# Terascale-All-sensing-Research-Studio/MOV-SLAM

Hardware: AMD Instinct MI355X
Metric: local-BA iterations/sec (50 KF x 20k MapPoint window) (higher is better)
Workload: dtype f64; 1 GPU; LocalBundleAdjustment 50 KF + 10 fixed x 20000 MapPoints, E=110510 mono edges, Huber on, 10 LM iterations (cfg3, seed 1003); one window per GPU; parallelism=1 window

## Files before the change

### mov-slam_amd/csrc/coarse_level.h

```cpp
#pragma once
#include <hip/hip_runtime.h>

#include <type_traits>

#include "device_math.h"
#include "device_types.h"
#include "handoff.h"

namespace movba {

#ifndef MOVBA_COARSE_EXTRAPOLATE
#define MOVBA_COARSE_EXTRAPOLATE 1
#endif

template <int kT, int kNC, int kPA>
__device__ __forceinline__ void coarse_build(const DevWindow &w, const PcgParams &pp, int trial, double lambda, double *sm, bool extrapolate)
{
    double *Ac = sm;
    double *gj = Ac + kNC * kNC;
    int &s_bad = *reinterpret_cast<int *>(gj + 9 * kNC + 2);
    const int tid = threadIdx.x;
    const int nf = w.nfree;
#ifdef MOVBA_CLOCK_STAMP
    unsigned long long cst_last = __builtin_amdgcn_s_memtime();
#define COARSE_STAMP(k) do { const unsigned long long _t = __builtin_amdgcn_s_memtime(); if (tid == 0) w.ctrl->dbg_seg2[k] += _t - cst_last; cst_last = _t; } while (0)
#else
#define COARSE_STAMP(k) do { } while (0)
#endif
    const double *part = w.part, *part_ = part;
    double *blocks = w.blocks_c;
    if (tid == 0) s_bad = 0;
    for (int idx = tid; idx < kNC * kNC; idx += kT) Ac[idx] = 0.0;

    const int ndiag = nf * 36;
    for (int idx = tid; idx < w.n_multi * 36; idx += kT) {
        const int m = idx / 36, k = idx - m * 36, pr = w.multi_pairs[m];
        double sacc = 0.0;
        for (int itx = w.pair_item_start[pr]; itx < w.pair_item_start[pr + 1]; ++itx) sacc += part[(size_t)itx * kPartStride + k];
        blocks[pr * 36 + k] = -sacc;
    }
    for (int base = tid; base < ndiag; base += 4 * kT) {
        int k[4], hu[4], i0[4], i1[4];
        double s[4] = { 0, 0, 0, 0 }, hp[4] = { 0, 0, 0, 0 };
        int nmax = 0;
#pragma unroll
        for (int m = 0; m < 4; ++m) {
            const int idx = min(base + m * kT, ndiag - 1);
            const int pr = idx / 36;
            k[m] = idx - pr * 36;
            const int a = k[m] / 6, b = k[m] - a * 6;
            hu[m] = 42 + (a <= b ? ut6(a, b) : ut6(b, a));
            i0[m] = w.pair_item_start[pr]; i1[m] = w.pair_item_start[pr + 1];
            nmax = max(nmax, i1[m] - i0[m]);
        }
        for (int o = 0; o < nmax; o += 6) {
            double sv[4][6], hv[4][6];
#pragma unroll
            for (int m = 0; m < 4; ++m)
#pragma unroll
                for (int u = 0; u < 6; ++u) {
                    const double *src = part + (size_t)min(i0[m] + o + u, i1[m] - 1) * kPartStride;
                    sv[m][u] = src[k[m]]; hv[m][u] = src[hu[m]];
                }
#pragma unroll
            for (int m = 0; m < 4; ++m)
#pragma unroll
                for (int u = 0; u < 6; ++u) { const bool in = i0[m] + o + u < i1[m]; s[m] += in ? sv[m][u] : 0.0; hp[m] += in ? hv[m][u] : 0.0; }
        }
#pragma unroll
        for (int m = 0; m < 4; ++m) {
            const int idx = base + m * kT;
            if (idx < ndiag) blocks[idx] = (hp[m] + ((k[m] % 7 == 0) ? lambda : 0.0)) - s[m];
        }
    }
    __syncthreads();
    COARSE_STAMP(2);
    double *aggc = gj;
    if (tid < kNC / kPA) {
        const int g0 = pp.wave_row0[tid], g1 = pp.wave_row0[tid + 1];
        aggc[tid] = g0 + 0.5 * (g1 - g0 - 1); aggc[kNC / kPA + tid] = 1.0 / fmax(1.0, 0.5 * (g1 - g0));
    }
    int *tent = reinterpret_cast<int *>(gj + 9 * kNC + 8), *tij = tent + w.cblk_ptr[w.n_cblk];
    for (int q = tid; q < w.cblk_ptr[w.n_cblk]; q += kT) { tent[q] = w.cblk_ent[q]; tij[q] = w.cblk_ij[q]; }
    __syncthreads();
    const int nw = w.n_cblk * 6;
    const bool split = 2 * nw <= kT;
    auto walk = [&](int cb, int a, int part, double (&s00)[6], double (&s01)[6], double (&s10)[6], double (&s11)[6]) {
        const int g = w.cblk_g[cb], h = w.cblk_h[cb];
        const double cg = aggc[g], ch = aggc[h], ig = aggc[kNC / kPA + g], ih = aggc[kNC / kPA + h];
        int t0 = w.cblk_ptr[cb], t1 = w.cblk_ptr[cb + 1];
        if (split) {
            const int n = t1 - t0, front = min(n, (((n + 1) >> 1) + 7) & ~7);
            if (part == 0) t1 = t0 + front; else t0 += front;
        }
#pragma unroll
        for (int m = 0; m < 6; ++m) s00[m] = s01[m] = s10[m] = s11[m] = 0.0;
        for (int t = t0; t < t1; t += 8) {
            int pk[8], ij[8];
            double v[8][6];
#pragma unroll
            for (int u = 0; u < 8; ++u) { const int tt = min(t + u, t1 - 1); pk[u] = tent[tt]; ij[u] = tij[tt]; }
#pragma unroll
            for (int u = 0; u < 8; ++u) {
                const int e = pk[u];
                const double *src = (e & 1) ? part_ + (size_t)(e >> 2) * kPartStride : blocks + (size_t)(e >> 2) * 36;
                const int o0 = (e & 2) ? a : a * 6, st = (e & 2) ? 6 : 1;
#pragma unroll
                for (int m = 0; m < 6; ++m) v[u][m] = src[o0 + st * m];
            }
#pragma unroll
            for (int u = 0; u < 8; ++u) {
                const bool in = t + u < t1;
                const double sgn = in ? ((pk[u] & 1) ? -1.0 : 1.0) : 0.0;
                const double pi = ((ij[u] >> 16) - cg) * ig, pj = ((ij[u] & 0xffff) - ch) * ih;
#pragma unroll
                for (int m = 0; m < 6; ++m) {
                    const double x = sgn * v[u][m];
                    s00[m] += x; s01[m] += pj * x; s10[m] += pi * x; s11[m] += pi * pj * x;
                }
            }
        }
        return Ac + (g * kPA + a) * kNC + h * kPA;
    };
    if (split) {
        const bool active = tid < 2 * nw;
        const int half = tid >= nw, wi = tid - half * nw;
        double s00[6], s01[6], s10[6], s11[6];
        double *dst = nullptr;
        if (active) dst = walk(wi / 6, wi - (wi / 6) * 6, half, s00, s01, s10, s11);
        if (active && !half) {
#pragma unroll
            for (int m = 0; m < 6; ++m) { dst[m] = s00[m]; dst[6 + m] = s01[m]; dst[6 * kNC + m] = s10[m]; dst[6 * kNC + 6 + m] = s11[m]; }
        }
        __syncthreads();
        if (active && half) {
#pragma unroll
            for (int m = 0; m < 6; ++m) { dst[m] += s00[m]; dst[6 + m] += s01[m]; dst[6 * kNC + m] += s10[m]; dst[6 * kNC + 6 + m] += s11[m]; }
        }
    } else {
        for (int wi = tid; wi < nw; wi += kT) {
            double s00[6], s01[6], s10[6], s11[6];
            double *dst = walk(wi / 6, wi - (wi / 6) * 6, 0, s00, s01, s10, s11);
#pragma unroll
            for (int m = 0; m < 6; ++m) { dst[m] = s00[m]; dst[6 + m] = s01[m]; dst[6 * kNC + m] = s10[m]; dst[6 * kNC + 6 + m] = s11[m]; }
        }
    }
    __syncthreads();
    if (tid < kNC) {
        const int g = tid / kPA, d = (tid - g * kPA) / 6, nrows = pp.wave_row0[g + 1] - pp.wave_row0[g];
        if (nrows == 0 || (d == 1 && nrows < 2)) {
            for (int j = 0; j < kNC; ++j) { Ac[tid * kNC + j] = 0.0; Ac[j * kNC + tid] = 0.0; }
        }
    }
    __syncthreads();
    if (tid < kNC) {
        const int g = tid / kPA, d = (tid - g * kPA) / 6, nrows = pp.wave_row0[g + 1] - pp.wave_row0[g];
        if (nrows == 0 || (d == 1 && nrows < 2)) Ac[tid * kNC + tid] = 1.0;
    }
    __syncthreads();
    if (extrapolate) {
        double *prev = w.ac_prev;
        const double lam_prev = prev[kNC * kNC], trial_prev = prev[kNC * kNC + 1];
        double gamma = 0.0;
        if (trial >= 1 && trial_prev == (double)(trial - 1) && lambda != lam_prev && MOVBA_COARSE_EXTRAPOLATE) {
            gamma = (lambda * (1.0 / 3.0) - lambda) / (lambda - lam_prev);
            gamma = fmin(fmax(gamma, -1.0), 1.0 / 3.0);
            if (!isfinite(gamma)) gamma = 0.0;
        }
        constexpr int kPer = kNC * kNC / kT;
        static_assert(kPer * kT == kNC * kNC, "one pass");
        double pv[kPer];
#pragma unroll
        for (int u = 0; u < kPer; ++u) pv[u] = prev[tid + u * kT];
        __syncthreads();
#pragma unroll
        for (int u = 0; u < kPer; ++u) {
            const double a = Ac[tid + u * kT];
            prev[tid + u * kT] = a;
            if (gamma != 0.0) Ac[tid + u * kT] = a + gamma * (a - pv[u]);
        }
        if (tid == 0) { prev[kNC * kNC] = lambda; prev[kNC * kNC + 1] = (double)trial; }
        __syncthreads();
    }

    COARSE_STAMP(3);
    static_assert(kNC == 96 && kT == 512, "tile layout written for 96 x 96 on 512 threads");
    double *dsc = gj + 8 * kNC + 2;
    double *pvs = gj + 8 * kNC;
    if (tid < kNC) { const double d = Ac[tid * kNC + tid]; dsc[tid] = (d > 0.0 && isfinite(d)) ? rsqrt(d) : 0.0; if (!(d > 0.0) || !isfinite(d)) s_bad = 1; }
    __syncthreads();
    const int rg = tid >> 4, cg = tid & 15;
    double t[3][6];
#pragma unroll
    for (int r = 0; r < 3; ++r)
#pragma unroll
        for (int q = 0; q < 6; ++q) t[r][q] = Ac[(3 * rg + r) * kNC + 6 * cg + q] * dsc[3 * rg + r] * dsc[6 * cg + q];
    unsigned live = 0;
    for (int q = 0; q < kNC / 6; ++q) {
        const int nrows = pp.wave_row0[(q >> 1) + 1] - pp.wave_row0[q >> 1];
        if (!(nrows == 0 || ((q & 1) && nrows < 2))) live |= 1u << q;
    }
    __syncthreads();
    auto publish = [&](auto Ctag, int gq, int buf) {
        constexpr int C = decltype(Ctag)::value;
        constexpr int lr0 = C % 3, lr1 = (C + 1) % 3;
        const int rg0 = 2 * gq + C / 3, rg1 = 2 * gq + (C + 1) / 3;
        double *R1 = gj + buf * 4 * kNC, *C1 = R1 + kNC, *R2 = C1 + kNC, *C2 = R2 + kNC;
        if (rg == rg0) {
#pragma unroll
            for (int q = 0; q < 6; ++q) R1[6 * cg + q] = t[lr0][q] + ((cg == gq && q == C) ? 1.0 : 0.0);
        }
        if (rg == rg1) {
#pragma unroll
            for (int q = 0; q < 6; ++q) R2[6 * cg + q] = t[lr1][q];
        }
        if (cg == gq) {
#pragma unroll
            for (int r = 0; r < 3; ++r) { C1[3 * rg + r] = t[r][C] - ((rg == rg0 && r == lr0) ? 1.0 : 0.0); C2[3 * rg + r] = t[r][C + 1]; }
        }
        if (rg == rg0 && cg == gq) pvs[buf] = t[lr0][C];
    };
    int kk = live ? __builtin_ctz(live) : kNC / 6;
    if (kk < kNC / 6) publish(std::integral_constant<int, 0>{}, kk, 0);
    __syncthreads();
    bool bad = s_bad != 0;
    int buf = 0;
    auto pair_step = [&](auto Ctag, int gq) -> bool {
        constexpr int C = decltype(Ctag)::value;
        constexpr int lr1 = (C + 1) % 3;
        const int k = 6 * gq + C, rg1 = 2 * gq + (C + 1) / 3;
        const double *R1 = gj + buf * 4 * kNC, *C1 = R1 + kNC, *R2 = C1 + kNC, *C2 = R2 + kNC;
        const double p1 = pvs[buf];
        const double o12 = R1[k + 1], o21 = C1[k + 1], q22 = R2[k + 1];
        double r1[6], r2[6], c1[3], c2[3];
#pragma unroll
        for (int q = 0; q < 6; ++q) { r1[q] = R1[6 * cg + q]; r2[q] = R2[6 * cg + q]; }
#pragma unroll
        for (int r = 0; r < 3; ++r) { c1[r] = C1[3 * rg + r]; c2[r] = C2[3 * rg + r]; }
        if (!(p1 > 0.0) || !isfinite(p1)) return false;
        double ip1 = __builtin_amdgcn_rcp(p1);
        ip1 = ip1 * (2.0 - p1 * ip1);
        ip1 = ip1 * (2.0 - p1 * ip1);
        const double s12 = o12 * ip1;
        const double p2 = q22 - o21 * s12;
        if (!(p2 > 0.0) || !isfinite(p2)) return false;
        double ip2 = __builtin_amdgcn_rcp(p2);
        ip2 = ip2 * (2.0 - p2 * ip2);
        ip2 = ip2 * (2.0 - p2 * ip2);
#pragma unroll
        for (int q = 0; q < 6; ++q) {
            r1[q] *= ip1;
            r2[q] = ((r2[q] - o21 * r1[q]) + ((cg == gq && q == C + 1) ? 1.0 : 0.0)) * ip2;
        }
#pragma unroll
        for (int r = 0; r < 3; ++r) c2[r] = (c2[r] - c1[r] * s12) - ((rg == rg1 && r == lr1) ? 1.0 : 0.0);
#pragma unroll
        for (int r = 0; r < 3; ++r)
#pragma unroll
            for (int q = 0; q < 6; ++q) { t[r][q] -= c1[r] * r1[q]; t[r][q] -= c2[r] * r2[q]; }
        return true;
    };
    while (kk < kNC / 6 && !bad) {
        const unsigned later = kk < 31 ? (live & ~((2u << kk) - 1u)) : 0u;
        const int next = later ? __builtin_ctz(later) : kNC / 6;
        if (!pair_step(std::integral_constant<int, 0>{}, kk)) { bad = true; break; }
        publish(std::integral_constant<int, 2>{}, kk, buf ^ 1);
        __syncthreads(); buf ^= 1;
        if (!pair_step(std::integral_constant<int, 2>{}, kk)) { bad = true; break; }
        publish(std::integral_constant<int, 4>{}, kk, buf ^ 1);
        __syncthreads(); buf ^= 1;
        if (!pair_step(std::integral_constant<int, 4>{}, kk)) { bad = true; break; }
        if (next < kNC / 6) publish(std::integral_constant<int, 0>{}, next, buf ^ 1);
        __syncthreads(); buf ^= 1;
        kk = next;
    }
    if (bad && tid == 0) s_bad = 1;
    __syncthreads();
    COARSE_STAMP(4);
    float *dst = w.aci + (size_t)(trial & 1) * kNC * kNC;
#pragma unroll
    for (int r = 0; r < 3; ++r)
#pragma unroll
        for (int q = 0; q < 6; ++q) dst[(3 * rg + r) * kNC + 6 * cg + q] = (float)(t[r][q] * dsc[3 * rg + r] * dsc[6 * cg + q]);
    __syncthreads();
    if (tid == 0) w.aci_tag[trial & 1] = s_bad ? -1 : trial;
    COARSE_STAMP(5);
}

}
```

Measured before the change: 9509 LM iterations/s.

## Replace pairwise Gauss-Jordan coarse inversion with blocked panel inversion using f64 MFMA

Replaces the register-tiled, pivot-pair Gauss-Jordan inversion of the 96x96 coarse matrix with a blocked 16-wide panel algorithm. Each panel is eliminated by two waves using cross-lane reads, then the trailing update runs as rank-16 updates through f64 MFMA 16x16x4 instructions. The goal is fewer barriers per pivot (two per 16 columns instead of one per two columns) and matrix-core throughput for the update. In exchange it operates in place on shared memory, skips panels only when all their pivot groups are dead, and changes rounding order.

```diff
diff --git a/mov-slam_amd/csrc/coarse_level.h b/mov-slam_amd/csrc/coarse_level.h
--- a/mov-slam_amd/csrc/coarse_level.h
+++ b/mov-slam_amd/csrc/coarse_level.h
@@ -12,6 +12,89 @@
 #ifndef MOVBA_COARSE_EXTRAPOLATE
 #define MOVBA_COARSE_EXTRAPOLATE 1
 #endif
+
+template <int kT, int kNC>
+__device__ __forceinline__ bool coarse_invert(unsigned live)
+{
+    extern __shared__ __attribute__((aligned(16))) double sm[];
+    double *Ac = sm, *gj = Ac + kNC * kNC;
+    int &s_bad = *reinterpret_cast<int *>(gj + 9 * kNC + 2);
+    const int tid = threadIdx.x;
+    static_assert(kNC == 96 && kT == 512, "panel layout written for 96 x 96 on 512 threads");
+    constexpr int kPB = 16, kNP = kNC / kPB;
+    double *dsc = gj + 8 * kNC + 2;
+    if (tid < kNC) { const double d = Ac[tid * kNC + tid]; dsc[tid] = (d > 0.0 && isfinite(d)) ? rsqrt(d) : 0.0; if (!(d > 0.0) || !isfinite(d)) s_bad = 1; }
+    __syncthreads();
+    for (int idx = tid; idx < kNC * kNC; idx += kT) { const int i = idx / kNC; Ac[idx] *= dsc[i] * dsc[idx - i * kNC]; }
+    __syncthreads();
+    const int gwv = __builtin_amdgcn_readfirstlane(tid >> 6), gln = tid & 63;
+    bool bad = false;
+#pragma unroll 1
+    for (int pn = 0; pn < kNP; ++pn) {
+        const int c0 = kPB * pn;
+        if (!((live >> (c0 / 6)) & ((1u << ((c0 + kPB - 1) / 6 - c0 / 6 + 1)) - 1u))) continue;
+        if (gwv < 2) {
+            const int m = gln - kPB + 48 * gwv;
+            const bool has_row = gln < kPB || m < kNC - kPB;
+            const int ri = gln < kPB ? c0 + gln : (has_row ? (m < c0 ? m : m + kPB) : c0);
+            const bool writes = has_row && (gwv == 0 || gln >= kPB);
+            double2 *rowp = reinterpret_cast<double2 *>(Ac + ri * kNC + c0);
+            double v[kPB];
+#pragma unroll
+            for (int c = 0; c < kPB; c += 2) { const double2 x = rowp[c >> 1]; v[c] = x.x; v[c + 1] = x.y; }
+#pragma unroll
+            for (int kk = 0; kk < kPB; ++kk) {
+                if (!((live >> ((c0 + kk) / 6)) & 1u)) continue;
+                const double p = readlane_f64(v[kk], kk);
+                if (!(p > 0.0) || !isfinite(p)) bad = true;
+                double ip = __builtin_amdgcn_rcp(p);
+                ip = ip * (2.0 - p * ip);
+                ip = ip * (2.0 - p * ip);
+                const bool isk = gln == kk;
+                const double tk = (isk ? 1.0 : v[kk]) * ip;
+#pragma unroll
+                for (int c4 = 0; c4 < kPB; c4 += 4) {
+                    double s[4];
+#pragma unroll
+                    for (int c = c4; c < c4 + 4; ++c) s[c - c4] = c == kk ? 0.0 : readlane_f64(v[c], kk);
+#pragma unroll
+                    for (int c = c4; c < c4 + 4; ++c)
+                        if (c != kk) v[c] = (isk ? 0.0 : v[c]) - tk * s[c - c4];
+                    __builtin_amdgcn_sched_barrier(0);
+                }
+                v[kk] = tk;
+            }
+            if (writes) {
+#pragma unroll
+                for (int c = 0; c < kPB; c += 2) rowp[c >> 1] = make_double2(v[c], v[c + 1]);
+            }
+        }
+        __syncthreads();
+        if (gwv < kNP - 1) {
+            const int jb = gwv < pn ? gwv : gwv + 1;
+            const double *bp = Ac + (c0 + (gln >> 4)) * kNC + kPB * jb + (gln & 15);
+            double bv[4];
+#pragma unroll
+            for (int q = 0; q < 4; ++q) bv[q] = bp[4 * q * kNC];
+#pragma unroll 1
+            for (int ib = 0; ib < kNP; ++ib) {
+                const double *ap = Ac + (kPB * ib + (gln & 15)) * kNC + c0 + (gln >> 4);
+                double *cp = Ac + (kPB * ib + (gln >> 4)) * kNC + kPB * jb + (gln & 15);
+                typedef double acc4 __attribute__((ext_vector_type(4)));
+                acc4 acc = { cp[0], cp[4 * kNC], cp[8 * kNC], cp[12 * kNC] };
+                if (ib == pn) acc = acc4{ 0.0, 0.0, 0.0, 0.0 };
+#pragma unroll
+                for (int q = 0; q < 4; ++q) acc = __builtin_amdgcn_mfma_f64_16x16x4f64(-ap[4 * q], bv[q], acc, 0, 0, 0);
+                cp[0] = acc.x; cp[4 * kNC] = acc.y; cp[8 * kNC] = acc.z; cp[12 * kNC] = acc.w;
+            }
+        }
+        __syncthreads();
+    }
+    bad = __any(bad);
+    if (bad && gln == 0) s_bad = 1;
+    __syncthreads();
+    return s_bad != 0;
+}
 
 template <int kT, int kNC, int kPA>
 __device__ __forceinline__ void coarse_build(const DevWindow &w, const PcgParams &pp, int trial, double lambda, double *sm, bool extrapolate)
@@ -184,106 +267,18 @@
     }
 
     COARSE_STAMP(3);
-    static_assert(kNC == 96 && kT == 512, "tile layout written for 96 x 96 on 512 threads");
-    double *dsc = gj + 8 * kNC + 2;
-    double *pvs = gj + 8 * kNC;
-    if (tid < kNC) { const double d = Ac[tid * kNC + tid]; dsc[tid] = (d > 0.0 && isfinite(d)) ? rsqrt(d) : 0.0; if (!(d > 0.0) || !isfinite(d)) s_bad = 1; }
-    __syncthreads();
-    const int rg = tid >> 4, cg = tid & 15;
-    double t[3][6];
-#pragma unroll
-    for (int r = 0; r < 3; ++r)
-#pragma unroll
-        for (int q = 0; q < 6; ++q) t[r][q] = Ac[(3 * rg + r) * kNC + 6 * cg + q] * dsc[3 * rg + r] * dsc[6 * cg + q];
     unsigned live = 0;
     for (int q = 0; q < kNC / 6; ++q) {
         const int nrows = pp.wave_row0[(q >> 1) + 1] - pp.wave_row0[q >> 1];
         if (!(nrows == 0 || ((q & 1) && nrows < 2))) live |= 1u << q;
     }
-    __syncthreads();
-    auto publish = [&](auto Ctag, int gq, int buf) {
-        constexpr int C = decltype(Ctag)::value;
-        constexpr int lr0 = C % 3, lr1 = (C + 1) % 3;
-        const int rg0 = 2 * gq + C / 3, rg1 = 2 * gq + (C + 1) / 3;
-        double *R1 = gj + buf * 4 * kNC, *C1 = R1 + kNC, *R2 = C1 + kNC, *C2 = R2 + kNC;
-        if (rg == rg0) {
-#pragma unroll
-            for (int q = 0; q < 6; ++q) R1[6 * cg + q] = t[lr0][q] + ((cg == gq && q == C) ? 1.0 : 0.0);
-        }
-        if (rg == rg1) {
-#pragma unroll
-            for (int q = 0; q < 6; ++q) R2[6 * cg + q] = t[lr1][q];
-        }
-        if (cg == gq) {
-#pragma unroll
-            for (int r = 0; r < 3; ++r) { C1[3 * rg + r] = t[r][C] - ((rg == rg0 && r == lr0) ? 1.0 : 0.0); C2[3 * rg + r] = t[r][C + 1]; }
-        }
-        if (rg == rg0 && cg == gq) pvs[buf] = t[lr0][C];
-    };
-    int kk = live ? __builtin_ctz(live) : kNC / 6;
-    if (kk < kNC / 6) publish(std::integral_constant<int, 0>{}, kk, 0);
-    __syncthreads();
-    bool bad = s_bad != 0;
-    int buf = 0;
-    auto pair_step = [&](auto Ctag, int gq) -> bool {
-        constexpr int C = decltype(Ctag)::value;
-        constexpr int lr1 = (C + 1) % 3;
-        const int k = 6 * gq + C, rg1 = 2 * gq + (C + 1) / 3;
-        const double *R1 = gj + buf * 4 * kNC, *C1 = R1 + kNC, *R2 = C1 + kNC, *C2 = R2 + kNC;
-        const double p1 = pvs[buf];
-        const double o12 = R1[k + 1], o21 = C1[k + 1], q22 = R2[k + 1];
-        double r1[6], r2[6], c1[3], c2[3];
-#pragma unroll
-        for (int q = 0; q < 6; ++q) { r1[q] = R1[6 * cg + q]; r2[q] = R2[6 * cg + q]; }
-#pragma unroll
-        for (int r = 0; r < 3; ++r) { c1[r] = C1[3 * rg + r]; c2[r] = C2[3 * rg + r]; }
-        if (!(p1 > 0.0) || !isfinite(p1)) return false;
-        double ip1 = __builtin_amdgcn_rcp(p1);
-        ip1 = ip1 * (2.0 - p1 * ip1);
-        ip1 = ip1 * (2.0 - p1 * ip1);
-        const double s12 = o12 * ip1;
-        const double p2 = q22 - o21 * s12;
-        if (!(p2 > 0.0) || !isfinite(p2)) return false;
-        double ip2 = __builtin_amdgcn_rcp(p2);
-        ip2 = ip2 * (2.0 - p2 * ip2);
-        ip2 = ip2 * (2.0 - p2 * ip2);
-#pragma unroll
-        for (int q = 0; q < 6; ++q) {
-            r1[q] *= ip1;
-            r2[q] = ((r2[q] - o21 * r1[q]) + ((cg == gq && q == C + 1) ? 1.0 : 0.0)) * ip2;
-        }
-#pragma unroll
-        for (int r = 0; r < 3; ++r) c2[r] = (c2[r] - c1[r] * s12) - ((rg == rg1 && r == lr1) ? 1.0 : 0.0);
-#pragma unroll
-        for (int r = 0; r < 3; ++r)
-#pragma unroll
-            for (int q = 0; q < 6; ++q) { t[r][q] -= c1[r] * r1[q]; t[r][q] -= c2[r] * r2[q]; }
-        return true;
-    };
-    while (kk < kNC / 6 && !bad) {
-        const unsigned later = kk < 31 ? (live & ~((2u << kk) - 1u)) : 0u;
-        const int next = later ? __builtin_ctz(later) : kNC / 6;
-        if (!pair_step(std::integral_constant<int, 0>{}, kk)) { bad = true; break; }
-        publish(std::integral_constant<int, 2>{}, kk, buf ^ 1);
-        __syncthreads(); buf ^= 1;
-        if (!pair_step(std::integral_constant<int, 2>{}, kk)) { bad = true; break; }
-        publish(std::integral_constant<int, 4>{}, kk, buf ^ 1);
-        __syncthreads(); buf ^= 1;
-        if (!pair_step(std::integral_constant<int, 4>{}, kk)) { bad = true; break; }
-        if (next < kNC / 6) publish(std::integral_constant<int, 0>{}, next, buf ^ 1);
-        __syncthreads(); buf ^= 1;
-        kk = next;
-    }
-    if (bad && tid == 0) s_bad = 1;
-    __syncthreads();
+    const bool inv_bad = coarse_invert<kT, kNC>(live);
+    const double *dsc = gj + 8 * kNC + 2;
     COARSE_STAMP(4);
     float *dst = w.aci + (size_t)(trial & 1) * kNC * kNC;
-#pragma unroll
-    for (int r = 0; r < 3; ++r)
-#pragma unroll
-        for (int q = 0; q < 6; ++q) dst[(3 * rg + r) * kNC + 6 * cg + q] = (float)(t[r][q] * dsc[3 * rg + r] * dsc[6 * cg + q]);
-    __syncthreads();
-    if (tid == 0) w.aci_tag[trial & 1] = s_bad ? -1 : trial;
+    for (int idx = tid; idx < kNC * kNC; idx += kT) { const int i = idx / kNC; dst[idx] = (float)(Ac[idx] * dsc[i] * dsc[idx - i * kNC]); }
+    __syncthreads();
+    if (tid == 0) w.aci_tag[trial & 1] = inv_bad ? -1 : trial;
     COARSE_STAMP(5);
 }
 
```

New measurement: 8050 LM iterations/s. 15.3% lower.
